# pxl-th/SLAM.jl

Hardware: AMD Instinct MI355X
Metric: frames/sec KITTI-05 stereo @1k kpts; local-BA ms/iter for 50-KF window (higher is better)
Workload: dtype f64

## Files before the change

### slam.jl_amd/csrc/pyramid.hip

```cpp
#include "common.hpp"
#include <cmath>
#include <cstdlib>
#include <mutex>
#include <tuple>
#include <utility>

#define LINE_THREADS 64

struct PlaneSet {
    double *p[4];
    const double *nrm[4];
    int coef[4];
    int fill0[4];
    const double *sq[4];
    int n;
    size_t zs;
};
#define PS_PICK(ps, f, pl) ((pl) == 0 ? (ps).f[0] : (pl) == 1 ? (ps).f[1] : (pl) == 2 ? (ps).f[2] : (ps).f[3])
__device__ __forceinline__ double *ps_plane(const PlaneSet &ps, int pl) { return PS_PICK(ps, p, pl) + (size_t)blockIdx.z * ps.zs; }
__device__ __forceinline__ const double *ps_nrm(const PlaneSet &ps, int pl) { return PS_PICK(ps, nrm, pl); }
__device__ __forceinline__ int ps_coef(const PlaneSet &ps, int pl) { return PS_PICK(ps, coef, pl); }
__device__ __forceinline__ bool ps_fill0(const PlaneSet &ps, int pl) { return PS_PICK(ps, fill0, pl) != 0; }
__device__ __forceinline__ const double *ps_sq(const PlaneSet &ps, int pl) { const double *q = PS_PICK(ps, sq, pl); return q ? q + (size_t)blockIdx.z * ps.zs : nullptr; }

// ... 1103 lines not shown
                for (int e = 0; e < hr; e++) { acc = (r0 + e == 0) ? c[e] : acc + c[e]; c[e] = acc; }
            }
        }
        if (w + 1 < nwh) {
            while (flag_ld(&s_done[w + 1]) + 2 <= cb) __builtin_amdgcn_s_sleep(1);
            if (lane < CF_W) carry_out[(cb & 1) * CF_W + lane] = acc;
            __builtin_amdgcn_fence(__ATOMIC_RELEASE, "workgroup", "local");
            if (lane == 0) flag_st(&s_ready[w], cb + 1);
        }
        else if (SEG && seg + 1 < nseg) {
            if (lane < CF_W && x0 + lane < W) __hip_atomic_store(xc_out + x0 + lane, acc, __ATOMIC_RELAXED, __HIP_MEMORY_SCOPE_AGENT);
            asm volatile("s_waitcnt vmcnt(0)" ::: "memory");
            if (lane == 0) __hip_atomic_store(xf_out, cb + 1, __ATOMIC_RELAXED, __HIP_MEMORY_SCOPE_AGENT);
        }
        __builtin_amdgcn_fence(__ATOMIC_RELEASE, "wavefront"); __builtin_amdgcn_wave_barrier();
        if (lane < hr) {
            ldsd *c = Cb + lane;
            if (wc == CF_W && cb > 0) {
                double v[CF_W];
#pragma unroll
                for (int j = 0; j < CF_W; j++) v[j] = c[j * CF_LS];
#pragma unroll
                for (int j = 0; j < CF_W; j++) { rcarry = rcarry + v[j]; v[j] = rcarry; }
#pragma unroll
                for (int j = 0; j < CF_W; j++) c[j * CF_LS] = v[j];
            } else {
                for (int j = 0; j < wc; j++) { rcarry = (cb == 0 && j == 0) ? c[j * CF_LS] : rcarry + c[j * CF_LS]; c[j * CF_LS] = rcarry; }
            }
        }
        __builtin_amdgcn_fence(__ATOMIC_RELEASE, "wavefront"); __builtin_amdgcn_wave_barrier();
#pragma unroll
        for (int sub = 0; sub < 4; sub++) {
            const int rb = r0 + sub * 16;
            if (rb < H) {
#pragma unroll
                for (int r = 0; r < 4; r++) {
                    const int col = x0 + 8 * r + cg, row = rb + 2 * rp;
                    const v2d q = *(const ldsv2 *)(Cb + (8 * r + cg) * CF_LS + sub * 16 + 2 * rp);
                    double *g = plane + ((size_t)(x0 + 8 * r) * P + rb) + voff;
                    if (col < W) {
                        if (row + 1 < H) __builtin_nontemporal_store(q, (v2d *)g);
                        else if (row < H) g[0] = q.x;
                    }
                }
            }
        }
        __builtin_amdgcn_fence(__ATOMIC_RELEASE, "wavefront"); __builtin_amdgcn_wave_barrier();
    }
    if (SEG && w == 0 && seg > 0 && lane == 0) __hip_atomic_store(xf_in, 0, __ATOMIC_RELAXED, __HIP_MEMORY_SCOPE_AGENT);
}

#define RC_CW 16
#define RC_LDS_DOUBLES (RC_CW * CF_LS + 2 * RC_CW)
__global__ __launch_bounds__(CF_MAXW * 64) void k_rows_cum(PlaneSet ps, int H, int W, int P, IIRPair cf, double *ck)
{
    extern __shared__ __attribute__((aligned(16))) double rc_lds[];
    __shared__ int s_ready[CF_MAXW], s_done[CF_MAXW];
    const int pl = blockIdx.y, lane = threadIdx.x & 63, w = threadIdx.x >> 6, nw = blockDim.x >> 6;
    typedef __attribute__((address_space(3))) double ldsd;
    typedef __attribute__((address_space(3))) v2d ldsv2;
    ldsd *Cb = (ldsd *)rc_lds + (size_t)w * RC_LDS_DOUBLES;
    ldsd *carry_out = Cb + RC_CW * CF_LS;
    const ldsd *carry_in = carry_out - RC_LDS_DOUBLES;
    auto flag_ld = [](int *f) { return __hip_atomic_load(f, __ATOMIC_RELAXED, __HIP_MEMORY_SCOPE_WORKGROUP); };
    auto flag_st = [](int *f, int v) { __hip_atomic_store(f, v, __ATOMIC_RELAXED, __HIP_MEMORY_SCOPE_WORKGROUP); };
    if (lane == 0) { flag_st(&s_ready[w], 0); flag_st(&s_done[w], 0); }
    __syncthreads();
    const int y = w * 64 + lane;
    const bool live = y < H;
    const size_t nlines = (size_t)gridDim.z * gridDim.y * blockDim.x;
    ck += ((size_t)blockIdx.z * gridDim.y + pl) * blockDim.x;
    const unsigned lid = threadIdx.x;
    double *plane = ps_plane(ps, pl);
    const unsigned yo = (unsigned)(live ? y : H - 1);
    double *p = plane + yo;
    const long s = P;
    const int n = W;
    const IIRCoef &k = ps_coef(ps, pl) == 0 ? cf.c[0] : cf.c[1];
    const bool fill0 = ps_fill0(ps, pl);
    const double a1 = k.a1, a2 = k.a2, a3 = k.a3, scale = k.scale;
    const double x0 = p[0];
    const double iminus = fill0 ? 0.0 : x0, iplus = fill0 ? 0.0 : p[(long)(n - 1) * s];
    const double uminus = iminus / k.inv1masum;
    const double o0 = ((x0 + a1 * uminus) + a2 * uminus) + a3 * uminus;
    const double o1 = ((p[s] + a1 * o0) + a2 * uminus) + a3 * uminus;
    const double o2 = ((p[2 * s] + a1 * o1) + a2 * o0) + a3 * uminus;
    const int m = n - 6, nb = (m + CK_B - 1) / CK_B;
    double w3 = o0, w2 = o1, w1 = o2;
    double cur[CK_B], nxt[CK_B];
    auto load_x = [&](int j, double *buf) {
        const int c0 = 3 + j * CK_B, len = n - c0;
        if (len >= CK_B) {
#pragma unroll
            for (int e = 0; e < CK_B; e++) buf[e] = RCK_LD(plane + (size_t)(c0 + e) * P + yo);
        } else {
#pragma unroll
            for (int e = 0; e < CK_B; e++) buf[e] = e < len ? plane[(size_t)(c0 + e) * P + yo] : 0.0;
        }
    };
    const int nfull = (n - 3) / CK_B, rem = (n - 3) - nfull * CK_B;
    load_x(0, cur);
    for (int j = 0; j < nfull; j++) {
        load_x(j + 1, nxt);
        if (j > 0 && j < nb) { double *c = ck + ((size_t)j * 3) * nlines + lid; CK_ST(c, w1); CK_ST(c + nlines, w2); CK_ST(c + 2 * nlines, w3); }
#pragma unroll
        for (int e = 0; e < CK_B; e++) { const double t = ((cur[e] + a1 * w1) + a2 * w2) + a3 * w3; w3 = w2; w2 = w1; w1 = t; }
#pragma unroll
        for (int e = 0; e < CK_B; e++) cur[e] = nxt[e];
    }
    {
        if (nfull > 0 && nfull < nb) { double *c = ck + ((size_t)nfull * 3) * nlines + lid; CK_ST(c, w1); CK_ST(c + nlines, w2); CK_ST(c + 2 * nlines, w3); }
#pragma unroll
        for (int e = 0; e < CK_B; e++)
            if (e < rem) { const double t = ((cur[e] + a1 * w1) + a2 * w2) + a3 * w3; w3 = w2; w2 = w1; w1 = t; }
    }
    const bool have_last = nfull == nb - 1;
    const double uplus = iplus / k.inv1masum, vplus = uplus / k.inv1mbsum;
    const double d0 = w1 - uplus, d1 = w2 - uplus, d2 = w3 - uplus;
    const double vr0 = ((k.M[0] * d0 + k.M[1] * d1) + k.M[2] * d2) + vplus;
    const double vr1 = ((k.M[3] * d0 + k.M[4] * d1) + k.M[5] * d2) + vplus;
    const double vr2 = ((k.M[6] * d0 + k.M[7] * d1) + k.M[8] * d2) + vplus;
    const double vA = vr0;
    const double vB = ((w2 + a1 * vA) + a2 * vr1) + a3 * vr2;
    const double vC = ((w3 + a1 * vB) + a2 * vA) + a3 * vr1;
    double v1 = vC, v2 = vB, v3 = vA;
    __builtin_amdgcn_fence(__ATOMIC_RELEASE, "workgroup"); __builtin_amdgcn_fence(__ATOMIC_ACQUIRE, "workgroup");
    double f1n = 0, f2n = 0, f3n = 0, f1 = 0, f2 = 0, f3 = 0;
    auto load_ck = [&](int j, double &g1, double &g2, double &g3) {
        if (j > 0) { const double *c = ck + ((size_t)j * 3) * nlines + lid; g1 = CK_LD(c); g2 = CK_LD(c + nlines); g3 = CK_LD(c + 2 * nlines); }
        else { g1 = o2; g2 = o1; g3 = o0; }
    };
    auto store_ack = [&](int j) { double *c = ck + ((size_t)j * 3) * nlines + lid; CK_ST(c, v1); CK_ST(c + nlines, v2); CK_ST(c + 2 * nlines, v3); };
    if (nb > 1) {
        const int j = nb - 1, len = m - j * CK_B;
        if (!have_last) load_x(j, cur);
        load_ck(j, f1, f2, f3);
        load_x(j - 1, nxt); load_ck(j - 1, f1n, f2n, f3n);
#pragma unroll
        for (int e = 0; e < CK_B; e++)
            if (e < len) { const double t = ((cur[e] + a1 * f1) + a2 * f2) + a3 * f3; f3 = f2; f2 = f1; f1 = t; cur[e] = t; }
        store_ack(j);
#pragma unroll
        for (int e = CK_B - 1; e >= 0; e--)
            if (e < len) { const double t = ((cur[e] + a1 * v1) + a2 * v2) + a3 * v3; v3 = v2; v2 = v1; v1 = t; }
#pragma unroll
        for (int e = 0; e < CK_B; e++) cur[e] = nxt[e];
        f1 = f1n; f2 = f2n; f3 = f3n;
    }
    for (int j = nb - 2; j >= 1; j--) {
        load_x(j - 1, nxt); load_ck(j - 1, f1n, f2n, f3n);
#pragma unroll
        for (int e = 0; e < CK_B; e++) { const double t = ((cur[e] + a1 * f1) + a2 * f2) + a3 * f3; f3 = f2; f2 = f1; f1 = t; cur[e] = t; }
        store_ack(j);
#pragma unroll
        for (int e = CK_B - 1; e >= 0; e--) { const double t = ((cur[e] + a1 * v1) + a2 * v2) + a3 * v3; v3 = v2; v2 = v1; v1 = t; }
#pragma unroll
        for (int e = 0; e < CK_B; e++) cur[e] = nxt[e];
        f1 = f1n; f2 = f2n; f3 = f3n;
    }
    if (nb > 0) store_ack(0);
    __builtin_amdgcn_fence(__ATOMIC_RELEASE, "workgroup"); __builtin_amdgcn_fence(__ATOMIC_ACQUIRE, "workgroup");
    double rcarry = -0.0;
    int hk = 0;
    auto cum_half = [&](int x0c, int wc) {
        __builtin_amdgcn_fence(__ATOMIC_RELEASE, "wavefront"); __builtin_amdgcn_wave_barrier();
        double acc = -0.0;
        if (w > 0) {
            while (flag_ld(&s_ready[w - 1]) <= hk) __builtin_amdgcn_s_sleep(1);
            __builtin_amdgcn_fence(__ATOMIC_ACQUIRE, "workgroup", "local");
            if (lane < RC_CW) acc = carry_in[(hk & 1) * RC_CW + lane];
            __builtin_amdgcn_fence(__ATOMIC_RELEASE, "workgroup", "local");
            if (lane == 0) flag_st(&s_done[w], hk + 1);
        }
        __builtin_amdgcn_fence(__ATOMIC_RELEASE, "wavefront"); __builtin_amdgcn_wave_barrier();
        if (lane < wc) {
            ldsd *c = Cb + lane * CF_LS;
#pragma unroll
            for (int g = 0; g < 4; g++) {
                double v[16];
#pragma unroll
                for (int j = 0; j < 8; j++) { const v2d q = *(const ldsv2 *)(c + 16 * g + 2 * j); v[2 * j] = q.x; v[2 * j + 1] = q.y; }
#pragma unroll
                for (int e = 0; e < 16; e++) { acc = acc + v[e]; v[e] = acc; }
#pragma unroll
                for (int j = 0; j < 8; j++) { const v2d t2 = {v[2 * j], v[2 * j + 1]}; *(ldsv2 *)(c + 16 * g + 2 * j) = t2; }
            }
        }
        if (w + 1 < nw) {
            while (flag_ld(&s_done[w + 1]) + 2 <= hk) __builtin_amdgcn_s_sleep(1);
            if (lane < RC_CW) carry_out[(hk & 1) * RC_CW + lane] = acc;
            __builtin_amdgcn_fence(__ATOMIC_RELEASE, "workgroup", "local");
            if (lane == 0) flag_st(&s_ready[w], hk + 1);
        }
        hk++;
        __builtin_amdgcn_fence(__ATOMIC_RELEASE, "wavefront"); __builtin_amdgcn_wave_barrier();
        double *q = plane + (size_t)x0c * P;
        if (wc == RC_CW) {
            double r[RC_CW];
#pragma unroll
            for (int j = 0; j < RC_CW; j++) r[j] = Cb[j * CF_LS + lane];
#pragma unroll
            for (int j = 0; j < RC_CW; j++) { rcarry = rcarry + r[j]; r[j] = rcarry; }
            if (live) {
#pragma unroll
                for (int j = 0; j < RC_CW; j++) RCK_ST(q + (size_t)j * P + yo, r[j]);
            }
        } else {
            for (int j = 0; j < wc; j++) { rcarry = rcarry + Cb[j * CF_LS + lane]; if (live) q[(size_t)j * P + yo] = rcarry; }
        }
        __builtin_amdgcn_fence(__ATOMIC_RELEASE, "wavefront"); __builtin_amdgcn_wave_barrier();
    };
    auto put = [&](int col, double v) { Cb[col * CF_LS + lane] = v; };
    double pv0 = 0, pv1 = 0, pv2 = 0;
    f1 = o2; f2 = o1; f3 = o0;
    if (nb > 0) {
        load_x(0, cur);
        { const double *c = ck + lid; v1 = CK_LD(c); v2 = CK_LD(c + nlines); v3 = CK_LD(c + 2 * nlines); }
    }
    for (int j = 0; j < nb; j++) {
        const int len = m - j * CK_B;
        double g1n = 0, g2n = 0, g3n = 0;
        if (len >= CK_B) {
#pragma unroll
            for (int e = 0; e < CK_B; e++) { const double t = ((cur[e] + a1 * f1) + a2 * f2) + a3 * f3; f3 = f2; f2 = f1; f1 = t; cur[e] = t; }
#pragma unroll
            for (int e = CK_B - 1; e >= 0; e--) { const double t = ((cur[e] + a1 * v1) + a2 * v2) + a3 * v3; v3 = v2; v2 = v1; v1 = t; cur[e] = t * scale; }
        } else {
#pragma unroll
            for (int e = 0; e < CK_B; e++)
                if (e < len) { const double t = ((cur[e] + a1 * f1) + a2 * f2) + a3 * f3; f3 = f2; f2 = f1; f1 = t; cur[e] = t; }
#pragma unroll
            for (int e = CK_B - 1; e >= 0; e--)
                if (e < len) { const double t = ((cur[e] + a1 * v1) + a2 * v2) + a3 * v3; v3 = v2; v2 = v1; v1 = t; cur[e] = t * scale; }
        }
        if (j == 0) {
            double t = ((o2 + a1 * v1) + a2 * v2) + a3 * v3; v3 = v2; v2 = v1; v1 = t; pv2 = t * scale;
            t = ((o1 + a1 * v1) + a2 * v2) + a3 * v3; v3 = v2; v2 = v1; v1 = t; pv1 = t * scale;
            t = ((o0 + a1 * v1) + a2 * v2) + a3 * v3; pv0 = t * scale;
        }
        if (j + 1 < nb) {
            load_x(j + 1, nxt);
            const double *c = ck + ((size_t)(j + 1) * 3) * nlines + lid; g1n = CK_LD(c); g2n = CK_LD(c + nlines); g3n = CK_LD(c + 2 * nlines);
        }
        const int x0 = j * CK_B;
        if (j + 1 < nb) {
            put(0, pv0); put(1, pv1); put(2, pv2);
#pragma unroll
            for (int e = 0; e < RC_CW - 3; e++) put(3 + e, cur[e]);
            cum_half(x0, RC_CW);
#pragma unroll
            for (int e = RC_CW - 3; e < CK_B - 3; e++) put(e + 3 - RC_CW, cur[e]);
            cum_half(x0 + RC_CW, RC_CW);
            pv0 = cur[CK_B - 3]; pv1 = cur[CK_B - 2]; pv2 = cur[CK_B - 1];
        } else {
            const double *c = ck + ((size_t)j * 3) * nlines + lid;
            const double t0 = CK_LD(c) * scale, t1 = CK_LD(c + nlines) * scale, t2 = CK_LD(c + 2 * nlines) * scale;
            const int tot = len + 6;
            for (int h = 0; h * RC_CW < tot; h++) {
                const int lo = h * RC_CW;
                auto putc = [&](int col, double v) { if (col >= lo && col < lo + RC_CW) put(col - lo, v); };
                putc(0, pv0); putc(1, pv1); putc(2, pv2);
#pragma unroll
                for (int e = 0; e < CK_B; e++) if (e < len) putc(3 + e, cur[e]);
                putc(len + 3, t0); putc(len + 4, t1); putc(len + 5, t2);
                cum_half(x0 + lo, min(RC_CW, tot - lo));
            }
        }
#pragma unroll
        for (int e = 0; e < CK_B; e++) cur[e] = nxt[e];
        v1 = g1n; v2 = g2n; v3 = g3n;
    }
}

#define PAR_T 1024
#define PAR_SLMAX 16
#define PAR_G 8
struct SegPow { double P[2][PAR_G][9]; double Plast[2][9]; };

__device__ __forceinline__ void mv3(const double *P, double &a, double &b, double &c, double za, double zb, double zc)
{
    const double n1 = __builtin_fma(P[0], a, __builtin_fma(P[1], b, __builtin_fma(P[2], c, za)));
    const double n2 = __builtin_fma(P[3], a, __builtin_fma(P[4], b, __builtin_fma(P[5], c, zb)));
    const double n3 = __builtin_fma(P[6], a, __builtin_fma(P[7], b, __builtin_fma(P[8], c, zc)));
    a = n1; b = n2; c = n3;
}

template <int ZG, int ZL, int GG, int GL, int ZN, int GN, class Slot>
__device__ __forceinline__ void fold_entry(const SegPow &sp, int cs, double (*Z)[ZN], double (*GT)[GN],
                                           int l, int k, bool has, Slot slot, double s0a, double s0b, double s0c,
                                           double &ea, double &eb, double &ec)
{
    const int q = k % PAR_G, grp = k / PAR_G;
    const double *P1 = sp.P[cs][0], *P8 = sp.P[cs][PAR_G - 1];
    double a = 0.0, b = 0.0, c = 0.0;
    if (has) for (int i = 0; i < q; i++) { const int s = slot(grp * PAR_G + i); mv3(P1, a, b, c, Z[0][s * ZG + l * ZL], Z[1][s * ZG + l * ZL], Z[2][s * ZG + l * ZL]); }
    if (has && q == PAR_G - 1) {
        double ta = a, tb = b, tc = c; const int s = slot(k);
        mv3(P1, ta, tb, tc, Z[0][s * ZG + l * ZL], Z[1][s * ZG + l * ZL], Z[2][s * ZG + l * ZL]);
        GT[0][grp * GG + l * GL] = ta; GT[1][grp * GG + l * GL] = tb; GT[2][grp * GG + l * GL] = tc;
    }
    __syncthreads();
    double Sa = s0a, Sb = s0b, Sc = s0c;
    if (has) {
        for (int h = 0; h < grp; h++) mv3(P8, Sa, Sb, Sc, GT[0][h * GG + l * GL], GT[1][h * GG + l * GL], GT[2][h * GG + l * GL]);
        if (q > 0) mv3(sp.P[cs][q - 1], Sa, Sb, Sc, 0.0, 0.0, 0.0);
    }
    ea = Sa + a; eb = Sb + b; ec = Sc + c;
}

template <bool COLS, int T = PAR_T, int LPW = 8>
__global__ __launch_bounds__(T) void k_iir_seg(PlaneSet ps, const double *src0, int H, int W, int P, IIRPair cf, SegPow sp, int SL, int cum_mask)
{
    if (src0) src0 += (size_t)blockIdx.z * ps.zs;
    constexpr int NSEG = T / LPW, ZN = T + 8, GN = T / PAR_G + 16;
    constexpr int ZG = COLS ? 1 : LPW, ZL = COLS ? NSEG + 1 : 1, GG = COLS ? 1 : LPW, GL = COLS ? NSEG / PAR_G + 2 : 1;
    __shared__ double Z[3][ZN];
    __shared__ double GT[3][GN];
    __shared__ double Fin[3][LPW];
    const int t = threadIdx.x, l = COLS ? t / NSEG : t % LPW, g = COLS ? t % NSEG : t / LPW, pl = blockIdx.y;
    const int nlines = COLS ? W : H, n = COLS ? H : W;
    const int line = blockIdx.x * LPW + l;
    const bool valid = line < nlines;
    const int lc = valid ? line : nlines - 1;
    const long stride = COLS ? 1 : P;
    const size_t off = COLS ? (size_t)lc * P : (size_t)lc;
    double *dstp = ps_plane(ps, pl) + off;
// ... 731 lines not shown
                        else B.launch((k_rows_tol<32, 2 * RT_NS, RT_R>), gr, bd, 0, LN_MAIN, ra, H, W, P, cf, spr);
                        return;
                    }
#define RT_GO(SLV) B.launch((k_rows_tol<SLV, RT_NS, RT_R>), gr, bd, 0, LN_MAIN, ra, H, W, P, cf, spr)
                    switch (slr_t) { case 4: RT_GO(4); break; case 6: RT_GO(6); break; case 8: RT_GO(8); break; case 10: RT_GO(10); break; case 12: RT_GO(12); break;
                                     case 16: RT_GO(16); break; case 20: RT_GO(20); break; case 24: RT_GO(24); break; case 32: RT_GO(32); break; default: RT_GO(40); break; }
#undef RT_GO
                };
                if (spans) { ProfScope span(ctx, "k_iir_rows"); go(); } else go();
                if (has_next && !rzf)
                    B.launch(k_resize, dim3(((size_t)p->H[l + 1] * p->W[l + 1] + 255) / 256, 1, S), dim3(256), 0, LN_MAIN,
                                       nextL, p->H[l + 1], p->W[l + 1], p->P[l + 1], (const double *)T, H, W, P, zs);
                return;
            }
        }
        else if (ck_cols) B.launch(k_iir_cols_ck, lines_grid(W, np, S), dim3(LINE_THREADS), 0, LN_MAIN, ps, src0, H, W, P, cf, p->ck);
        else if (topo) {
            B.launch(k_iir_cols<3>, lines_grid(W, 1, S), dim3(LINE_THREADS), 0, LN_MAIN, psT, src0, H, W, P, cf);
            B.launch(k_iir_cols<3>, lines_grid(W, 3, S), dim3(LINE_THREADS), 0, side, psQ, (const double *)nullptr, H, W, P, cf);
        }
        else if (S == 1) B.launch(k_iir_cols<3>, lines_grid(W, np, S), dim3(LINE_THREADS), 0, LN_MAIN, ps, src0, H, W, P, cf);
        else B.launch(k_iir_cols<2>, lines_grid(W, np, S), dim3(LINE_THREADS), 0, LN_MAIN, ps, src0, H, W, P, cf);
        const bool ck_rows = p->ck != nullptr && mode != 0 && W >= 64 && (size_t)Sall * np * H * W * 8 >= ck_min_bytes();
        static const bool no_rows_resize = getenv("SLAMHIP_NO_ROWS_RESIZE") != nullptr;
        const bool rz_odd_cand = ck_rows && has_next && (H & 1) != 0 && !no_rows_resize;
        bool rows_resize = ck_rows && has_next && (H & 1) == 0 && !no_rows_resize;
        bool rows_odd = false;
        RowResize rz = {};
        auto rz_decide = [&](int nplanes) {
            if (rz_odd_cand && nplanes == 1 && rz_odd_ok(p, l)) rows_resize = rows_odd = true;
            if (rows_resize) { rz.dst = nextL; rz.Hd = p->H[l + 1]; rz.Wd = p->W[l + 1]; rz.Pd = p->P[l + 1]; }
        };
        static const bool no_rows_cum = getenv("SLAMHIP_NO_ROWS_CUM") != nullptr;
        static const bool no_fused_cum = getenv("SLAMHIP_NO_FUSED_CUM") != nullptr;
        const int cf_bands = (H + 63) / 64;
        if (!topo && Sall >= 8 && mode != 0 && W >= 64 && cf_bands <= CF_MAXW && p->alloc->rck != nullptr && !no_rows_cum && !no_fused_cum) {
            B.fork();
            if (has_next) {
                PlaneSet pT = {}; pT.p[0] = ps.p[0]; pT.coef[0] = ps.coef[0]; pT.fill0[0] = ps.fill0[0]; pT.n = 1; pT.zs = zs;
                rz_decide(1);
                if (spans) { ProfScope span(ctx, "k_iir_rows");
                    if (ck_rows) launch_rows_ck(B, pT, 1, S, H, W, P, cf, p->ck, rz, rows_odd);
                    else B.launch(k_iir_rows, lines_grid(H, 1, S), dim3(LINE_THREADS), 0, LN_MAIN, pT, H, W, P, cf); }
                else if (ck_rows) launch_rows_ck(B, pT, 1, S, H, W, P, cf, p->ck, rz, rows_odd);
                else B.launch(k_iir_rows, lines_grid(H, 1, S), dim3(LINE_THREADS), 0, LN_MAIN, pT, H, W, P, cf);
                if (!rows_resize)
                    B.launch(k_resize, dim3(((size_t)p->H[l + 1] * p->W[l + 1] + 255) / 256, 1, S), dim3(256), 0, LN_MAIN,
                                       nextL, p->H[l + 1], p->W[l + 1], p->P[l + 1], (const double *)T, H, W, P, zs);
            }
            PlaneSet pq = {};
            for (int q = 0; q < 3; q++) { pq.p[q] = ps.p[np - 3 + q]; pq.coef[q] = ps.coef[np - 3 + q]; pq.fill0[q] = ps.fill0[np - 3 + q]; }
            pq.n = 3; pq.zs = zs;
            const size_t lds = (size_t)cf_bands * RC_LDS_DOUBLES * sizeof(double);
            B.launch(k_rows_cum, dim3(1, 3, S), dim3(cf_bands * 64), lds, LN_AUX, pq, H, W, P, cf, p->alloc->rck);
            return;
        }
        if (!topo) rz_decide(np);
        if (topo) {
            B.launch(k_iir_rows, lines_grid(H, 1, S), dim3(LINE_THREADS), 0, LN_MAIN, psT, H, W, P, cf);
            B.launch(k_iir_rows, lines_grid(H, 3, S), dim3(LINE_THREADS), 0, side, psQ, H, W, P, cf);
        }
        else if (spans) { ProfScope span(ctx, "k_iir_rows");
            if (ck_rows) launch_rows_ck(B, ps, np, S, H, W, P, cf, p->ck, rz, rows_odd);
            else B.launch(k_iir_rows, lines_grid(H, np, S), dim3(LINE_THREADS), 0, LN_MAIN, ps, H, W, P, cf); }
        else if (ck_rows) launch_rows_ck(B, ps, np, S, H, W, P, cf, p->ck, rz, rows_odd);
        else B.launch(k_iir_rows, lines_grid(H, np, S), dim3(LINE_THREADS), 0, LN_MAIN, ps, H, W, P, cf);
        if (!topo) B.fork();
        if (has_next && !rows_resize)
            B.launch(k_resize, dim3(((size_t)p->H[l + 1] * p->W[l + 1] + 255) / 256, 1, S), dim3(256), 0, LN_MAIN,
                               nextL, p->H[l + 1], p->W[l + 1], p->P[l + 1], (const double *)T, H, W, P, zs);
        const int cf_seg = cf_bands <= CF_MAXW ? 1 : (cf_bands + CF_SEGW - 1) / CF_SEGW;
        if (Sall >= 8 && !no_fused_cum && (cf_seg == 1 || (p->alloc->xc != nullptr && cf_seg <= p->alloc->xseg))) {
            const int nw = cf_seg == 1 ? cf_bands : CF_SEGW;
            const size_t lds = ((size_t)nw * CF_W * CF_LS + (size_t)nw * 2 * CF_W) * sizeof(double);
            const size_t xo = (size_t)z0 * 3 * (size_t)(cf_seg > 1 ? cf_seg - 1 : 1);
            if (cf_seg == 1) B.launch(k_cum_fused<false>, dim3(1, 3, S), dim3(nw * 64), lds, LN_AUX, pc, H, W, P, (double *)nullptr, (int *)nullptr);
            else B.launch(k_cum_fused<true>, dim3(cf_seg, 3, S), dim3(nw * 64), lds, LN_AUX, pc, H, W, P, p->alloc->xc + xo * W, p->alloc->xf + xo);
            return;
        }
        if (S == 1) B.launch(k_cum_cols<3>, lines_grid(W, 3, S), dim3(LINE_THREADS), 0, side_cum, pc, H, W, P);
        else B.launch(k_cum_cols<2>, lines_grid(W, 3, S), dim3(LINE_THREADS), 0, LN_AUX, pc, H, W, P);
        B.launch(k_cum_rows, lines_grid(H, 3, S), dim3(LINE_THREADS), 0, S == 1 ? side_cum : LN_AUX, pc, H, W, P);
    }
}


static void launch_build(slam_ctx *ctx, slam_pyr *p, int mode, const IIRPair &cf, BuildSink &B, bool spans, int S = 1, int src_kind = 0, bool target = false)
{
    bool fast = mode == 3;
    if (fast && (seg_len(p->H[0], PAR_T / 8) > PAR_SLMAX || seg_len(p->W[0], PAR_T / 8) > PAR_SLMAX)) fast = false;
    if (fast && S >= tol_batch_min_s()) fast = false;
    static const int chunk_mb = [] { const char *v = getenv("SLAMHIP_PYR_CHUNK_MB"); return v ? atoi(v) : 0; }();
    for (int l = 0; l < p->levels; l++) {
        int C = S;
        if (chunk_mb > 0 && S >= 8 && mode != 0) {
            const size_t per_image = (size_t)4 * p->P[l] * p->W[l] * 8;
            const size_t want = (size_t)chunk_mb << 20;
            if (per_image * S > 2 * want) { C = (int)std::max<size_t>(4, want / per_image); C = std::min(C, S); }
        }
        for (int z0 = 0; z0 < S; z0 += C) launch_level(ctx, p, mode, cf, B, spans, std::min(C, S - z0), src_kind, target, l, z0, S, fast);
    }
}

static bool level0_fused(const slam_pyr *p, int mode, int S)
{
    static const bool off = getenv("SLAMHIP_NO_COLS_FUSED") != nullptr || getenv("SLAMHIP_NO_SQ_FUSE") != nullptr || getenv("SLAMHIP_NO_CK_COLS") != nullptr ||
                            getenv("SLAMHIP_NO_FUSED_INGEST") != nullptr;
// ... 38 lines not shown
            hipError_t e = hipGraphCreate(&graph, 0);
            if (e == hipSuccess) {
                BuildSink B; B.graph = graph; B.forked = !chain;
                launch_build(ctx, p, mode, cf, B, false, S, src_kind & 15, target);
                e = B.err;
            }
            if (e == hipSuccess) e = hipGraphInstantiate(&exec, graph, nullptr, nullptr, 0);
            if (graph) (void)hipGraphDestroy(graph);
            if (e != hipSuccess) { (void)hipGetLastError(); p->graph_failed = true; exec = nullptr; }
            else { slam_pyr::Graph g; g.mode = mode; g.sigma = sigma; g.S = S; g.ckmin = ckmin; g.src_kind = src_kind; g.exec = exec; p->graphs.push_back(g); }
        }
        if (exec) HIP_TRY(ctx, hipGraphLaunch(exec, st));
    }
    if (!exec) { BuildSink B; B.st = st; launch_build(ctx, p, mode, cf, B, false, S, src_kind & 15, target); }
    HIP_TRY(ctx, hipGetLastError());
    return SLAM_OK;
}

static void ingest_dense(slam_ctx *ctx, slam_pyr *p, const double *image_dev)
{
    ImgPtrs ip = {}; ip.p[0] = image_dev;
    const size_t n = (size_t)p->H[0] * p->W[0];
    hipLaunchKernelGGL(k_gather_images, dim3((n + 255) / 256, 1, 1), dim3(256), 0, ctx->stream, ip, p->plane(0, 0), p->H[0], p->W[0], p->P[0], (size_t)0);
}

extern "C" {

static int pyr_create_n(slam_ctx *ctx, int H, int W, int pyramid_levels, int S, slam_pyr **out)
{
    ARG_TRY(ctx, ctx != nullptr && out != nullptr);
    ARG_TRY(ctx, H >= 4 && W >= 4 && pyramid_levels >= 0 && pyramid_levels + 1 <= SLAM_MAX_LEVELS && S >= 1 && S <= BATCH_MAX);
    HIP_TRY(ctx, hipSetDevice(ctx->device));
    int Hs[SLAM_MAX_LEVELS], Ws[SLAM_MAX_LEVELS], Ps[SLAM_MAX_LEVELS]; int64_t off[SLAM_MAX_LEVELS + 1];
    int64_t o = 0; int h = H, w = W;
    const int levels = pyramid_levels + 1;
    for (int l = 0; l < levels; l++) {
        if (h < 4 || w < 4) return slam_fail(ctx, SLAM_ERR_ARG, "slam_pyr_create: level %d is %dx%d, too small for the IIR kernel (needs > 3)", l, h, w);
        Hs[l] = h; Ws[l] = w; Ps[l] = (h + 15) & ~15; off[l] = o; o += (int64_t)Ps[l] * w;
        h = (h + 1) / 2; w = (w + 1) / 2;
    }
    off[levels] = o;
    slam_pyr::Alloc *al = new slam_pyr::Alloc();
    const size_t tail = (size_t)64 * Ps[0];
    hipError_t e = hipMalloc((void **)&al->base, ((size_t)o * 7 * S + tail) * 8);
    if (e != hipSuccess) { delete al; return slam_fail(ctx, SLAM_ERR_HIP, "slam_pyr_create: hipMalloc: %s", hipGetErrorString(e)); }
    e = hipMemsetAsync(al->base, 0, ((size_t)o * 7 * S + tail) * 8, ctx->stream);
    if (e == hipSuccess) e = slam_stream_wait(ctx->stream);
    if (e != hipSuccess) { (void)hipFree(al->base); delete al; return slam_fail(ctx, SLAM_ERR_HIP, "slam_pyr_create: memset: %s", hipGetErrorString(e)); }
    al->refs = S;
    if (S > 1 && hipMalloc((void **)&al->srctab, BATCH_MAX * sizeof(void *)) != hipSuccess) { (void)hipGetLastError(); al->srctab = nullptr; }
    {
        hipError_t ea = hipFuncSetAttribute((const void *)k_cum_fused<false>, hipFuncAttributeMaxDynamicSharedMemorySize, 150 * 1024);
        if (ea == hipSuccess) ea = hipFuncSetAttribute((const void *)k_cum_fused<true>, hipFuncAttributeMaxDynamicSharedMemorySize, 150 * 1024);
        if (ea == hipSuccess) ea = hipFuncSetAttribute((const void *)k_rows_cum, hipFuncAttributeMaxDynamicSharedMemorySize, 150 * 1024);
        if (ea != hipSuccess) { (void)hipFree(al->base); delete al; return slam_fail(ctx, SLAM_ERR_HIP, "slam_pyr_create: hipFuncSetAttribute(k_cum_fused): %s", hipGetErrorString(ea)); }
    }
    double *ckbuf = nullptr;
    if (S > 1) {
        const size_t lines = (size_t)S * 4 * (((size_t)Hs[0] + LINE_THREADS - 1) / LINE_THREADS) * LINE_THREADS;
        const size_t nbk = ((size_t)Ws[0] + CK_B - 1) / CK_B;
        const size_t lines_c = (size_t)S * 4 * (((size_t)Ws[0] + CF4_COLS - 1) / CF4_COLS) * LINE_THREADS;
        const size_t nbk_c = ((size_t)Hs[0] + 31) / 32 + 1;
        const size_t need = lines * nbk > lines_c * nbk_c ? lines * nbk : lines_c * nbk_c;
        if (hipMalloc((void **)&ckbuf, need * 3 * 8) != hipSuccess) { (void)hipGetLastError(); ckbuf = nullptr; }
        al->ck = ckbuf;
        if ((Hs[0] + 63) / 64 <= CF_MAXW) {
            const size_t lines_r = (size_t)S * 3 * (((size_t)Hs[0] + 63) / 64) * 64;
            if (hipMalloc((void **)&al->rck, lines_r * nbk * 3 * 8) != hipSuccess) { (void)hipGetLastError(); al->rck = nullptr; }
        }
        size_t wsum = 0; for (int l = 0; l < levels; l++) wsum += (size_t)Ws[l];
        if (hipMalloc((void **)&al->tot, (size_t)3 * S * wsum * 8) != hipSuccess) { (void)hipGetLastError(); al->tot = nullptr; }
        const int xbands = (Hs[0] + 63) / 64, xseg = xbands <= CF_MAXW ? 1 : (xbands + CF_SEGW - 1) / CF_SEGW;
        if (xseg > 1 && ctx->arch_ok) {
            const size_t nslot = (size_t)S * 3 * (xseg - 1);
            if (hipMalloc((void **)&al->xc, nslot * Ws[0] * 8) != hipSuccess) { (void)hipGetLastError(); al->xc = nullptr; }
            if (al->xc && (hipMalloc((void **)&al->xf, nslot * 4) != hipSuccess || hipMemset(al->xf, 0, nslot * 4) != hipSuccess)) { (void)hipGetLastError(); (void)hipFree(al->xc); al->xc = nullptr; al->xf = nullptr; }
            if (al->xc) al->xseg = xseg;
        }
    }
    for (int s = 0; s < S; s++) {
        slam_pyr *p = new slam_pyr();
        p->device = ctx->device; p->levels = levels;
        memcpy(p->H, Hs, sizeof Hs); memcpy(p->W, Ws, sizeof Ws); memcpy(p->P, Ps, sizeof Ps); memcpy(p->off, off, sizeof off);
        p->alloc = al;
        p->zstride = (size_t)o * 7;
        p->planes = al->base + (size_t)s * p->zstride;
        p->tmp = p->planes + (size_t)o * 6;
        p->batch_index = s; p->batch_size = S; p->ck = ckbuf;
        make_view(p);
        out[s] = p;
    }
    return SLAM_OK;
}

int slam_pyr_create(slam_ctx *ctx, int H, int W, int pyramid_levels, slam_pyr **out)
{
    return pyr_create_n(ctx, H, W, pyramid_levels, 1, out);
}

int slam_pyr_create_batch(slam_ctx *ctx, int H, int W, int pyramid_levels, int S, slam_pyr **out)
{
    return pyr_create_n(ctx, H, W, pyramid_levels, S, out);
}

int slam_pyr_update_batch_dev(slam_ctx *ctx, slam_pyr *const *pyrs, const double *const *images_dev, int S, int mode, double sigma, int sync)
{
    ARG_TRY(ctx, ctx != nullptr && pyrs != nullptr && images_dev != nullptr && S >= 1 && S <= BATCH_MAX && ((mode & ~SLAM_PYR_FLAGS) == 1 || (mode & ~SLAM_PYR_FLAGS) == 3) && sigma > 0);
// ... 150 lines not shown
```

Baseline: 23500.

## Add low-register k_rows_cum variant without prefetch for multi-round grids

Templates k_rows_cum on a prefetch flag. The non-prefetch variant drops the double-buffered next-block registers, uses raw buffer loads and stores with offsets (nontemporal for bulk plane traffic), recomputes the boundary terms instead of keeping them live, and uses a smaller scan group, all to fit three waves per EU. The host picks this variant when the 3*S blocks would need more than one round over the CUs, or when an environment override asks for it. The cost is less latency hiding per wave, since loads are no longer prefetched, and buffer size limits gate when the variant can be used.

```diff
diff --git a/slam.jl_amd/csrc/pyramid.hip b/slam.jl_amd/csrc/pyramid.hip
--- a/slam.jl_amd/csrc/pyramid.hip
+++ b/slam.jl_amd/csrc/pyramid.hip
@@ -1179,10 +1179,14 @@
 
 #define RC_CW 16
 #define RC_LDS_DOUBLES (RC_CW * CF_LS + 2 * RC_CW)
-__global__ __launch_bounds__(CF_MAXW * 64) void k_rows_cum(PlaneSet ps, int H, int W, int P, IIRPair cf, double *ck)
+#define RC_W3_MAXW 6
+template <bool PF>
+__global__ __launch_bounds__((PF ? CF_MAXW : RC_W3_MAXW) * 64) __attribute__((amdgpu_waves_per_eu(PF ? 1 : 3, PF ? 0 : 3)))
+void k_rows_cum(PlaneSet ps, int H, int W, int P, IIRPair cf, double *ck)
 {
     extern __shared__ __attribute__((aligned(16))) double rc_lds[];
     __shared__ int s_ready[CF_MAXW], s_done[CF_MAXW];
+    constexpr int RC_G = PF ? 16 : 8;
     const int pl = blockIdx.y, lane = threadIdx.x & 63, w = threadIdx.x >> 6, nw = blockDim.x >> 6;
     typedef __attribute__((address_space(3))) double ldsd;
     typedef __attribute__((address_space(3))) v2d ldsv2;
@@ -1201,6 +1205,20 @@
     double *plane = ps_plane(ps, pl);
     const unsigned yo = (unsigned)(live ? y : H - 1);
     double *p = plane + yo;
+    const unsigned yob = yo * (unsigned)sizeof(double);
+    typedef unsigned v2u __attribute__((ext_vector_type(2)));
+    __amdgpu_buffer_rsrc_t prs, crs;
+    if constexpr (!PF) {
+        prs = __builtin_amdgcn_make_buffer_rsrc(plane, 0, W * P * (int)sizeof(double), 0x00020000);
+        crs = __builtin_amdgcn_make_buffer_rsrc(ck, 0, (int)((3 * ((W - 6 + CK_B - 1) / CK_B) * nlines - ((size_t)blockIdx.z * gridDim.y + pl) * blockDim.x) * sizeof(double)), 0x00020000);
+    }
+    const unsigned lidb = lid * (unsigned)sizeof(double);
+    auto ckb_ld = [&](int slot) { return __builtin_bit_cast(double, __builtin_amdgcn_raw_buffer_load_b64(crs, lidb, (unsigned)slot * (unsigned)nlines * 8u, 0)); };
+    auto ckb_st = [&](int slot, double v) { __builtin_amdgcn_raw_buffer_store_b64(__builtin_bit_cast(v2u, v), crs, lidb, (unsigned)slot * (unsigned)nlines * 8u, 0); };
+    auto pl_ld = [&](int col) { return __builtin_bit_cast(double, __builtin_amdgcn_raw_buffer_load_b64(prs, yob, (unsigned)(col * P) * 8u, 0)); };
+    auto pl_ld_nt = [&](int col) { return __builtin_bit_cast(double, __builtin_amdgcn_raw_buffer_load_b64(prs, yob, (unsigned)(col * P) * 8u, 2)); };
+    auto pl_st = [&](int col, double v) { __builtin_amdgcn_raw_buffer_store_b64(__builtin_bit_cast(v2u, v), prs, yob, (unsigned)(col * P) * 8u, 0); };
+    auto pl_st_nt = [&](int col, double v) { __builtin_amdgcn_raw_buffer_store_b64(__builtin_bit_cast(v2u, v), prs, yob, (unsigned)(col * P) * 8u, 2); };
     const long s = P;
     const int n = W;
     const IIRCoef &k = ps_coef(ps, pl) == 0 ? cf.c[0] : cf.c[1];
@@ -1209,34 +1227,46 @@
     const double x0 = p[0];
     const double iminus = fill0 ? 0.0 : x0, iplus = fill0 ? 0.0 : p[(long)(n - 1) * s];
     const double uminus = iminus / k.inv1masum;
-    const double o0 = ((x0 + a1 * uminus) + a2 * uminus) + a3 * uminus;
-    const double o1 = ((p[s] + a1 * o0) + a2 * uminus) + a3 * uminus;
-    const double o2 = ((p[2 * s] + a1 * o1) + a2 * o0) + a3 * uminus;
+    double o0 = ((x0 + a1 * uminus) + a2 * uminus) + a3 * uminus;
+    double o1 = ((p[s] + a1 * o0) + a2 * uminus) + a3 * uminus;
+    double o2 = ((p[2 * s] + a1 * o1) + a2 * o0) + a3 * uminus;
     const int m = n - 6, nb = (m + CK_B - 1) / CK_B;
     double w3 = o0, w2 = o1, w1 = o2;
-    double cur[CK_B], nxt[CK_B];
+    double cur[CK_B], nxt[PF ? CK_B : 1];
     auto load_x = [&](int j, double *buf) {
         const int c0 = 3 + j * CK_B, len = n - c0;
         if (len >= CK_B) {
 #pragma unroll
-            for (int e = 0; e < CK_B; e++) buf[e] = RCK_LD(plane + (size_t)(c0 + e) * P + yo);
+            for (int e = 0; e < CK_B; e++) { if constexpr (PF) buf[e] = RCK_LD(plane + (size_t)(c0 + e) * P + yo); else buf[e] = pl_ld_nt(c0 + e); }
+        } else if constexpr (PF) {
+#pragma unroll
+            for (int e = 0; e < CK_B; e++) buf[e] = e < len ? plane[(size_t)(c0 + e) * P + yo] : 0.0;
         } else {
 #pragma unroll
-            for (int e = 0; e < CK_B; e++) buf[e] = e < len ? plane[(size_t)(c0 + e) * P + yo] : 0.0;
+            for (int e = 0; e < CK_B; e++) buf[e] = pl_ld(min(c0 + e, n - 1));
         }
     };
     const int nfull = (n - 3) / CK_B, rem = (n - 3) - nfull * CK_B;
-    load_x(0, cur);
+    if constexpr (PF) load_x(0, cur);
     for (int j = 0; j < nfull; j++) {
-        load_x(j + 1, nxt);
-        if (j > 0 && j < nb) { double *c = ck + ((size_t)j * 3) * nlines + lid; CK_ST(c, w1); CK_ST(c + nlines, w2); CK_ST(c + 2 * nlines, w3); }
+        if constexpr (PF) load_x(j + 1, nxt); else load_x(j, cur);
+        if (j > 0 && j < nb) {
+            if constexpr (PF) { double *c = ck + ((size_t)j * 3) * nlines + lid; CK_ST(c, w1); CK_ST(c + nlines, w2); CK_ST(c + 2 * nlines, w3); }
+            else { ckb_st(3 * j, w1); ckb_st(3 * j + 1, w2); ckb_st(3 * j + 2, w3); }
+        }
 #pragma unroll
         for (int e = 0; e < CK_B; e++) { const double t = ((cur[e] + a1 * w1) + a2 * w2) + a3 * w3; w3 = w2; w2 = w1; w1 = t; }
-#pragma unroll
-        for (int e = 0; e < CK_B; e++) cur[e] = nxt[e];
+        if constexpr (PF) {
+#pragma unroll
+            for (int e = 0; e < CK_B; e++) cur[e] = nxt[e];
+        }
     }
     {
-        if (nfull > 0 && nfull < nb) { double *c = ck + ((size_t)nfull * 3) * nlines + lid; CK_ST(c, w1); CK_ST(c + nlines, w2); CK_ST(c + 2 * nlines, w3); }
+        if constexpr (!PF) load_x(nfull, cur);
+        if (nfull > 0 && nfull < nb) {
+            if constexpr (PF) { double *c = ck + ((size_t)nfull * 3) * nlines + lid; CK_ST(c, w1); CK_ST(c + nlines, w2); CK_ST(c + 2 * nlines, w3); }
+            else { ckb_st(3 * nfull, w1); ckb_st(3 * nfull + 1, w2); ckb_st(3 * nfull + 2, w3); }
+        }
 #pragma unroll
         for (int e = 0; e < CK_B; e++)
             if (e < rem) { const double t = ((cur[e] + a1 * w1) + a2 * w2) + a3 * w3; w3 = w2; w2 = w1; w1 = t; }
@@ -1254,15 +1284,19 @@
     __builtin_amdgcn_fence(__ATOMIC_RELEASE, "workgroup"); __builtin_amdgcn_fence(__ATOMIC_ACQUIRE, "workgroup");
     double f1n = 0, f2n = 0, f3n = 0, f1 = 0, f2 = 0, f3 = 0;
     auto load_ck = [&](int j, double &g1, double &g2, double &g3) {
-        if (j > 0) { const double *c = ck + ((size_t)j * 3) * nlines + lid; g1 = CK_LD(c); g2 = CK_LD(c + nlines); g3 = CK_LD(c + 2 * nlines); }
+        if constexpr (!PF) { g1 = ckb_ld(3 * j); g2 = ckb_ld(3 * j + 1); g3 = ckb_ld(3 * j + 2); }
+        else if (j > 0) { const double *c = ck + ((size_t)j * 3) * nlines + lid; g1 = CK_LD(c); g2 = CK_LD(c + nlines); g3 = CK_LD(c + 2 * nlines); }
         else { g1 = o2; g2 = o1; g3 = o0; }
     };
-    auto store_ack = [&](int j) { double *c = ck + ((size_t)j * 3) * nlines + lid; CK_ST(c, v1); CK_ST(c + nlines, v2); CK_ST(c + 2 * nlines, v3); };
+    auto store_ack = [&](int j) {
+        if constexpr (PF) { double *c = ck + ((size_t)j * 3) * nlines + lid; CK_ST(c, v1); CK_ST(c + nlines, v2); CK_ST(c + 2 * nlines, v3); }
+        else { ckb_st(3 * j, v1); ckb_st(3 * j + 1, v2); ckb_st(3 * j + 2, v3); }
+    };
     if (nb > 1) {
         const int j = nb - 1, len = m - j * CK_B;
         if (!have_last) load_x(j, cur);
         load_ck(j, f1, f2, f3);
-        load_x(j - 1, nxt); load_ck(j - 1, f1n, f2n, f3n);
+        if constexpr (PF) { load_x(j - 1, nxt); load_ck(j - 1, f1n, f2n, f3n); }
 #pragma unroll
         for (int e = 0; e < CK_B; e++)
             if (e < len) { const double t = ((cur[e] + a1 * f1) + a2 * f2) + a3 * f3; f3 = f2; f2 = f1; f1 = t; cur[e] = t; }
@@ -1270,20 +1304,25 @@
 #pragma unroll
         for (int e = CK_B - 1; e >= 0; e--)
             if (e < len) { const double t = ((cur[e] + a1 * v1) + a2 * v2) + a3 * v3; v3 = v2; v2 = v1; v1 = t; }
-#pragma unroll
-        for (int e = 0; e < CK_B; e++) cur[e] = nxt[e];
-        f1 = f1n; f2 = f2n; f3 = f3n;
+        if constexpr (PF) {
+#pragma unroll
+            for (int e = 0; e < CK_B; e++) cur[e] = nxt[e];
+            f1 = f1n; f2 = f2n; f3 = f3n;
+        }
     }
     for (int j = nb - 2; j >= 1; j--) {
-        load_x(j - 1, nxt); load_ck(j - 1, f1n, f2n, f3n);
+        if constexpr (PF) { load_x(j - 1, nxt); load_ck(j - 1, f1n, f2n, f3n); }
+        else { load_x(j, cur); load_ck(j, f1, f2, f3); }
 #pragma unroll
         for (int e = 0; e < CK_B; e++) { const double t = ((cur[e] + a1 * f1) + a2 * f2) + a3 * f3; f3 = f2; f2 = f1; f1 = t; cur[e] = t; }
         store_ack(j);
 #pragma unroll
         for (int e = CK_B - 1; e >= 0; e--) { const double t = ((cur[e] + a1 * v1) + a2 * v2) + a3 * v3; v3 = v2; v2 = v1; v1 = t; }
-#pragma unroll
-        for (int e = 0; e < CK_B; e++) cur[e] = nxt[e];
-        f1 = f1n; f2 = f2n; f3 = f3n;
+        if constexpr (PF) {
+#pragma unroll
+            for (int e = 0; e < CK_B; e++) cur[e] = nxt[e];
+            f1 = f1n; f2 = f2n; f3 = f3n;
+        }
     }
     if (nb > 0) store_ack(0);
     __builtin_amdgcn_fence(__ATOMIC_RELEASE, "workgroup"); __builtin_amdgcn_fence(__ATOMIC_ACQUIRE, "workgroup");
@@ -1303,14 +1342,14 @@
         if (lane < wc) {
             ldsd *c = Cb + lane * CF_LS;
 #pragma unroll
-            for (int g = 0; g < 4; g++) {
-                double v[16];
-#pragma unroll
-                for (int j = 0; j < 8; j++) { const v2d q = *(const ldsv2 *)(c + 16 * g + 2 * j); v[2 * j] = q.x; v[2 * j + 1] = q.y; }
-#pragma unroll
-                for (int e = 0; e < 16; e++) { acc = acc + v[e]; v[e] = acc; }
-#pragma unroll
-                for (int j = 0; j < 8; j++) { const v2d t2 = {v[2 * j], v[2 * j + 1]}; *(ldsv2 *)(c + 16 * g + 2 * j) = t2; }
+            for (int g = 0; g < 64 / RC_G; g++) {
+                double v[RC_G];
+#pragma unroll
+                for (int j = 0; j < RC_G / 2; j++) { const v2d q = *(const ldsv2 *)(c + RC_G * g + 2 * j); v[2 * j] = q.x; v[2 * j + 1] = q.y; }
+#pragma unroll
+                for (int e = 0; e < RC_G; e++) { acc = acc + v[e]; v[e] = acc; }
+#pragma unroll
+                for (int j = 0; j < RC_G / 2; j++) { const v2d t2 = {v[2 * j], v[2 * j + 1]}; *(ldsv2 *)(c + RC_G * g + 2 * j) = t2; }
             }
         }
         if (w + 1 < nw) {
@@ -1323,82 +1362,118 @@
         __builtin_amdgcn_fence(__ATOMIC_RELEASE, "wavefront"); __builtin_amdgcn_wave_barrier();
         double *q = plane + (size_t)x0c * P;
         if (wc == RC_CW) {
-            double r[RC_CW];
-#pragma unroll
-            for (int j = 0; j < RC_CW; j++) r[j] = Cb[j * CF_LS + lane];
-#pragma unroll
-            for (int j = 0; j < RC_CW; j++) { rcarry = rcarry + r[j]; r[j] = rcarry; }
-            if (live) {
-#pragma unroll
-                for (int j = 0; j < RC_CW; j++) RCK_ST(q + (size_t)j * P + yo, r[j]);
+#pragma unroll
+            for (int g = 0; g < RC_CW; g += RC_G) {
+                double r[RC_G];
+#pragma unroll
+                for (int j = 0; j < RC_G; j++) r[j] = Cb[(g + j) * CF_LS + lane];
+#pragma unroll
+                for (int j = 0; j < RC_G; j++) { rcarry = rcarry + r[j]; r[j] = rcarry; }
+                if (live) {
+#pragma unroll
+                    for (int j = 0; j < RC_G; j++) { if constexpr (PF) RCK_ST(q + (size_t)(g + j) * P + yo, r[j]); else pl_st_nt(x0c + g + j, r[j]); }
+                }
             }
         } else {
-            for (int j = 0; j < wc; j++) { rcarry = rcarry + Cb[j * CF_LS + lane]; if (live) q[(size_t)j * P + yo] = rcarry; }
+            for (int j = 0; j < wc; j++) { rcarry = rcarry + Cb[j * CF_LS + lane]; if (live) { if constexpr (PF) q[(size_t)j * P + yo] = rcarry; else pl_st(x0c + j, rcarry); } }
         }
         __builtin_amdgcn_fence(__ATOMIC_RELEASE, "wavefront"); __builtin_amdgcn_wave_barrier();
     };
     auto put = [&](int col, double v) { Cb[col * CF_LS + lane] = v; };
     double pv0 = 0, pv1 = 0, pv2 = 0;
+    auto derive_o = [&]() {
+        const double xa = pl_ld(0), xb = pl_ld(1), xc = pl_ld(2);
+        const double um = (fill0 ? 0.0 : xa) / k.inv1masum;
+        o0 = ((xa + a1 * um) + a2 * um) + a3 * um;
+        o1 = ((xb + a1 * o0) + a2 * um) + a3 * um;
+        o2 = ((xc + a1 * o1) + a2 * o0) + a3 * um;
+    };
+    if constexpr (!PF) derive_o();
     f1 = o2; f2 = o1; f3 = o0;
-    if (nb > 0) {
-        load_x(0, cur);
-        { const double *c = ck + lid; v1 = CK_LD(c); v2 = CK_LD(c + nlines); v3 = CK_LD(c + 2 * nlines); }
+    if constexpr (PF) {
+        if (nb > 0) {
+            load_x(0, cur);
+            { const double *c = ck + lid; v1 = CK_LD(c); v2 = CK_LD(c + nlines); v3 = CK_LD(c + 2 * nlines); }
+        }
     }
     for (int j = 0; j < nb; j++) {
         const int len = m - j * CK_B;
         double g1n = 0, g2n = 0, g3n = 0;
+        if constexpr (!PF) {
+            load_x(j, cur);
+            v1 = ckb_ld(3 * j); v2 = ckb_ld(3 * j + 1); v3 = ckb_ld(3 * j + 2);
+        }
         if (len >= CK_B) {
 #pragma unroll
             for (int e = 0; e < CK_B; e++) { const double t = ((cur[e] + a1 * f1) + a2 * f2) + a3 * f3; f3 = f2; f2 = f1; f1 = t; cur[e] = t; }
 #pragma unroll
             for (int e = CK_B - 1; e >= 0; e--) { const double t = ((cur[e] + a1 * v1) + a2 * v2) + a3 * v3; v3 = v2; v2 = v1; v1 = t; cur[e] = t * scale; }
-        } else {
+        } else if constexpr (PF) {
 #pragma unroll
             for (int e = 0; e < CK_B; e++)
                 if (e < len) { const double t = ((cur[e] + a1 * f1) + a2 * f2) + a3 * f3; f3 = f2; f2 = f1; f1 = t; cur[e] = t; }
 #pragma unroll
             for (int e = CK_B - 1; e >= 0; e--)
                 if (e < len) { const double t = ((cur[e] + a1 * v1) + a2 * v2) + a3 * v3; v3 = v2; v2 = v1; v1 = t; cur[e] = t * scale; }
+        } else {
+#pragma unroll
+            for (int e = 0; e < CK_B; e++) { const double t = ((cur[e] + a1 * f1) + a2 * f2) + a3 * f3; f3 = f2; f2 = f1; f1 = t; cur[e] = t; }
+#pragma unroll
+            for (int e = CK_B - 1; e >= 0; e--) {
+                const double t = ((cur[e] + a1 * v1) + a2 * v2) + a3 * v3; const bool in = e < len;
+                v3 = in ? v2 : v3; v2 = in ? v1 : v2; v1 = in ? t : v1; cur[e] = t * scale;
+                asm volatile("" : "+v"(cur[e]));
+            }
         }
         if (j == 0) {
+            if constexpr (!PF) derive_o();
             double t = ((o2 + a1 * v1) + a2 * v2) + a3 * v3; v3 = v2; v2 = v1; v1 = t; pv2 = t * scale;
             t = ((o1 + a1 * v1) + a2 * v2) + a3 * v3; v3 = v2; v2 = v1; v1 = t; pv1 = t * scale;
             t = ((o0 + a1 * v1) + a2 * v2) + a3 * v3; pv0 = t * scale;
-        }
-        if (j + 1 < nb) {
-            load_x(j + 1, nxt);
-            const double *c = ck + ((size_t)(j + 1) * 3) * nlines + lid; g1n = CK_LD(c); g2n = CK_LD(c + nlines); g3n = CK_LD(c + 2 * nlines);
+            if constexpr (!PF) { put(0, pv0); put(1, pv1); put(2, pv2); }
+        }
+        if constexpr (PF) {
+            if (j + 1 < nb) {
+                load_x(j + 1, nxt);
+                const double *c = ck + ((size_t)(j + 1) * 3) * nlines + lid; g1n = CK_LD(c); g2n = CK_LD(c + nlines); g3n = CK_LD(c + 2 * nlines);
+            }
         }
         const int x0 = j * CK_B;
         if (j + 1 < nb) {
-            put(0, pv0); put(1, pv1); put(2, pv2);
+            if constexpr (PF) { put(0, pv0); put(1, pv1); put(2, pv2); }
 #pragma unroll
             for (int e = 0; e < RC_CW - 3; e++) put(3 + e, cur[e]);
             cum_half(x0, RC_CW);
 #pragma unroll
             for (int e = RC_CW - 3; e < CK_B - 3; e++) put(e + 3 - RC_CW, cur[e]);
             cum_half(x0 + RC_CW, RC_CW);
-            pv0 = cur[CK_B - 3]; pv1 = cur[CK_B - 2]; pv2 = cur[CK_B - 1];
+            if constexpr (PF) { pv0 = cur[CK_B - 3]; pv1 = cur[CK_B - 2]; pv2 = cur[CK_B - 1]; }
+            else { put(0, cur[CK_B - 3]); put(1, cur[CK_B - 2]); put(2, cur[CK_B - 1]); }
         } else {
             const double *c = ck + ((size_t)j * 3) * nlines + lid;
-            const double t0 = CK_LD(c) * scale, t1 = CK_LD(c + nlines) * scale, t2 = CK_LD(c + 2 * nlines) * scale;
+            double t0 = 0, t1 = 0, t2 = 0;
+            if constexpr (PF) { t0 = CK_LD(c) * scale; t1 = CK_LD(c + nlines) * scale; t2 = CK_LD(c + 2 * nlines) * scale; }
             const int tot = len + 6;
             for (int h = 0; h * RC_CW < tot; h++) {
                 const int lo = h * RC_CW;
                 auto putc = [&](int col, double v) { if (col >= lo && col < lo + RC_CW) put(col - lo, v); };
-                putc(0, pv0); putc(1, pv1); putc(2, pv2);
+                if constexpr (PF) { putc(0, pv0); putc(1, pv1); putc(2, pv2); }
 #pragma unroll
                 for (int e = 0; e < CK_B; e++) if (e < len) putc(3 + e, cur[e]);
+                if constexpr (!PF) {
+                    if (len + 5 >= lo && len + 3 < lo + RC_CW) { t0 = ckb_ld(3 * j) * scale; t1 = ckb_ld(3 * j + 1) * scale; t2 = ckb_ld(3 * j + 2) * scale; }
+                }
                 putc(len + 3, t0); putc(len + 4, t1); putc(len + 5, t2);
                 cum_half(x0 + lo, min(RC_CW, tot - lo));
             }
         }
-#pragma unroll
-        for (int e = 0; e < CK_B; e++) cur[e] = nxt[e];
-        v1 = g1n; v2 = g2n; v3 = g3n;
-    }
-}
-
+        if constexpr (PF) {
+#pragma unroll
+            for (int e = 0; e < CK_B; e++) cur[e] = nxt[e];
+            v1 = g1n; v2 = g2n; v3 = g3n;
+        }
+    }
+}
 #define PAR_T 1024
 #define PAR_SLMAX 16
 #define PAR_G 8
@@ -2236,7 +2311,14 @@
             for (int q = 0; q < 3; q++) { pq.p[q] = ps.p[np - 3 + q]; pq.coef[q] = ps.coef[np - 3 + q]; pq.fill0[q] = ps.fill0[np - 3 + q]; }
             pq.n = 3; pq.zs = zs;
             const size_t lds = (size_t)cf_bands * RC_LDS_DOUBLES * sizeof(double);
-            B.launch(k_rows_cum, dim3(1, 3, S), dim3(cf_bands * 64), lds, LN_AUX, pq, H, W, P, cf, p->alloc->rck);
+            static const char *rows_cum_w2 = getenv("SLAMHIP_ROWS_CUM_W2");
+            const size_t rc_ck_bytes = (size_t)3 * ((W - 6 + CK_B - 1) / CK_B) * ((size_t)S * 3 * cf_bands * 64) * sizeof(double);
+            const bool w3_can = cf_bands <= RC_W3_MAXW && (size_t)W * P * sizeof(double) < ((size_t)1 << 31) && rc_ck_bytes < ((size_t)1 << 31);
+            const int rc_cus = ctx->cus > 0 ? ctx->cus : ctx->dev_cus;
+            const bool second_round = rc_cus > 0 && (long)3 * S > (long)(8 / cf_bands) * rc_cus;
+            const bool w3 = w3_can && (rows_cum_w2 ? rows_cum_w2[0] == '0' : second_round);
+            if (w3) B.launch(k_rows_cum<false>, dim3(1, 3, S), dim3(cf_bands * 64), lds, LN_AUX, pq, H, W, P, cf, p->alloc->rck);
+            else B.launch(k_rows_cum<true>, dim3(1, 3, S), dim3(cf_bands * 64), lds, LN_AUX, pq, H, W, P, cf, p->alloc->rck);
             return;
         }
         if (!topo) rz_decide(np);
@@ -2381,7 +2463,8 @@
     {
         hipError_t ea = hipFuncSetAttribute((const void *)k_cum_fused<false>, hipFuncAttributeMaxDynamicSharedMemorySize, 150 * 1024);
         if (ea == hipSuccess) ea = hipFuncSetAttribute((const void *)k_cum_fused<true>, hipFuncAttributeMaxDynamicSharedMemorySize, 150 * 1024);
-        if (ea == hipSuccess) ea = hipFuncSetAttribute((const void *)k_rows_cum, hipFuncAttributeMaxDynamicSharedMemorySize, 150 * 1024);
+        if (ea == hipSuccess) ea = hipFuncSetAttribute((const void *)k_rows_cum<true>, hipFuncAttributeMaxDynamicSharedMemorySize, 150 * 1024);
+        if (ea == hipSuccess) ea = hipFuncSetAttribute((const void *)k_rows_cum<false>, hipFuncAttributeMaxDynamicSharedMemorySize, 150 * 1024);
         if (ea != hipSuccess) { (void)hipFree(al->base); delete al; return slam_fail(ctx, SLAM_ERR_HIP, "slam_pyr_create: hipFuncSetAttribute(k_cum_fused): %s", hipGetErrorString(ea)); }
     }
     double *ckbuf = nullptr;
```

New measurement: 23770, median of 4. +1.1%, better.
